# wcq99681-svg/YOLO-AD-Refine

Hardware: AMD Instinct MI355X
Metric: images/sec whole-node (640x640) fwd+bwd, YOLO-AD-Refine-n at 1/2/4/8 GPU (higher is better)
Workload: dtype bf16; 1 GPU; yolo11-701-YOLO-AD-Refine.yaml (n) train step bs=64/GPU 640x640, synthetic COCO-shape labels, TAL+DFL+CIoU/NWD loss, SGD+EMA; global_batch=64, img=640, parallelism=dp1, nms=not in the train step (measured in the inference leg at validator settings)

## Files before the change

### yolo-ad-refine_amd/csrc/adr_mlca.hip

```cpp
#include "adr_common.h"
#include <initializer_list>

namespace adr {

static constexpr int LS = 5;
__device__ __forceinline__ int a_s(int o, int in, int out) { return (int)(((long)o * in) / out); }
__device__ __forceinline__ int a_e(int o, int in, int out) { return (int)(((long)(o + 1) * in + out - 1) / out); }

template <typename T, int VW>
__global__ void __launch_bounds__(256) mlca_pool_kernel(const T* x, int xcs, int H, int W, int C, float* local) {
  __shared__ float red[256 * VW];
  const int p = blockIdx.x, n = blockIdx.y;
  const int i = p / LS, j = p % LS;
  const int hs = a_s(i, H, LS), he = a_e(i, H, LS), ws = a_s(j, W, LS), we = a_e(j, W, LS);
  const int bw = we - ws, cnt = (he - hs) * bw;
  const float inv = 1.f / (float)cnt;
  const int G = C / VW;
  for (int cb = 0; cb < G; cb += 256) {
    const int gn = min(256, G - cb), S = 256 / gn;
    const int cg = cb + threadIdx.x % gn, sp = threadIdx.x / gn, c0 = cg * VW;
    float s[VW];
#pragma unroll
    for (int e = 0; e < VW; ++e) s[e] = 0.f;
    if (sp < S)
// ... 270 lines not shown
    up_att<VW>(att + (long)n * LS * LS * C, C, h, w, H, W, c0, a);
    vload<T, VW>(dout + pix * dcs + c0, g);
#pragma unroll
    for (int e = 0; e < VW; ++e) g[e] *= a[e];
    const float* DL = dlocal + (long)n * LS * LS * C + c0;
    const int bic = h * LS / H, bjc = w * LS / W;
    const int bi0 = H < 2 * LS ? 0 : max(0, bic - 1), bi1 = H < 2 * LS ? LS - 1 : min(LS - 1, bic + 1);
    const int bj0 = W < 2 * LS ? 0 : max(0, bjc - 1), bj1 = W < 2 * LS ? LS - 1 : min(LS - 1, bjc + 1);
    for (int bi = bi0; bi <= bi1; ++bi) {
      const int hs = a_s(bi, H, LS), he = a_e(bi, H, LS);
      if (h < hs || h >= he) continue;
      for (int bj = bj0; bj <= bj1; ++bj) {
        const int ws = a_s(bj, W, LS), we = a_e(bj, W, LS);
        if (w < ws || w >= we) continue;
        const float inv = 1.f / (float)((he - hs) * (we - ws));
        const float* d = DL + (bi * LS + bj) * C;
#pragma unroll
        for (int e = 0; e < VW; ++e) g[e] += d[e] * inv;
      }
    }
    vstore<T, VW>(dy + pix * ocs + c0, g);
  }
}

__global__ void sum_rows_kernel(const float* part, int rows, int cols, float* out0, float* out1) {
  const int c = threadIdx.x;
  if (c >= cols) return;
  const float* p = part + (long)blockIdx.x * cols;
  float s = 0.f;
  for (int r = 0; r < rows; ++r) s += p[(long)r * 2 * cols + c];
  (blockIdx.x ? out1 : out0)[c] = s;
}

}

using namespace adr;

static bool mlca_vec(int dtype, int C, std::initializer_list<long> strides, std::initializer_list<const void*> ptrs) {
  const int vw = dtype == ADR_BF16 ? 8 : 4;
  if (C % vw) return false;
  for (long s : strides)
    if (s % vw) return false;
  for (const void* p : ptrs)
    if ((uintptr_t)p % 16) return false;
  return true;
}
static dim3 mlca_grid(long npix, int dtype, bool v, int C) {
  const int G = C / (v ? (dtype == ADR_BF16 ? 8 : 4) : 1);
  const long rpb = G <= 256 ? 256 / G : 1;
  long b = (npix + rpb - 1) / rpb;
  return dim3((unsigned)(b > 65536 ? 65536 : (b < 1 ? 1 : b)));
}
#define MLCA_DISPATCH(dtype, v, KERN, grid, ...)                                                  \
  do {                                                                                          \
    if ((dtype) == ADR_BF16) {                                                                  \
      using TT = __bf16;                                                                        \
      if (v) hipLaunchKernelGGL((KERN<TT, 8>), grid, dim3(256), 0, st, __VA_ARGS__);            \
      else hipLaunchKernelGGL((KERN<TT, 1>), grid, dim3(256), 0, st, __VA_ARGS__);              \
    } else {                                                                                    \
      using TT = float;                                                                         \
      if (v) hipLaunchKernelGGL((KERN<TT, 4>), grid, dim3(256), 0, st, __VA_ARGS__);            \
      else hipLaunchKernelGGL((KERN<TT, 1>), grid, dim3(256), 0, st, __VA_ARGS__);              \
    }                                                                                           \
  } while (0)

extern "C" int adr_mlca_fwd(int dtype, const void* y, int ycs, const void* res, int rcs, void* out, int ocs, int N,
                            int H, int W, int C, const float* wl, const float* wg, int k, float local_weight,
                            float* local, float* att, float* sig_l, float* sig_g, void* stream) {
  ADR_REQUIRE(k % 2 == 1 && k <= 15, "mlca: k=%d", k);
  ADR_REQUIRE(N >= 1 && H >= 1 && W >= 1 && C >= 1, "mlca_fwd: empty map N=%d H=%d W=%d C=%d", N, H, W, C);
  hipStream_t st = (hipStream_t)stream;
  const bool v = mlca_vec(dtype, C, {ycs, rcs, ocs}, {y, res, out});
  MLCA_DISPATCH(dtype, v, mlca_pool_kernel, dim3(LS * LS, N), (const TT*)y, ycs, H, W, C, local);
  size_t sm = 2 * C * sizeof(float);
  hipLaunchKernelGGL(mlca_att_kernel, dim3(N), dim3(256), sm, st, local, C, wl, wg, k, sig_l, sig_g);
  long natt = (long)N * LS * LS * C;
  hipLaunchKernelGGL(mlca_mix_kernel, dim3(cdiv(natt, 256)), dim3(256), 0, st, sig_l, sig_g, N, C, local_weight, att);
  MLCA_DISPATCH(dtype, v, mlca_apply_kernel, mlca_grid((long)N * H * W, dtype, v, C), (const TT*)y, ycs,
                (const TT*)res, rcs, att, (TT*)out, ocs, N, H, W, C);
  return check_launch("adr_mlca_fwd");
}

extern "C" size_t adr_mlca_bwd_workspace(int N, int C, int k) {
  return ((size_t)N * LS * LS * C * 2 + (size_t)N * k * 2 + (size_t)LS * C) * sizeof(float);
}

extern "C" int adr_mlca_bwd(int dtype, const void* y, int ycs, const void* dout, int dcs, void* dy, int ocs, int N,
                            int H, int W, int C, const float* wl, const float* wg, int k, float local_weight,
                            const float* local, const float* att, const float* sig_l, const float* sig_g, float* dwl,
                            float* dwg, float* ws, size_t ws_bytes, void* stream) {
  ADR_REQUIRE(N >= 1 && H >= 1 && W >= 1 && C >= 1, "mlca_bwd: empty map N=%d H=%d W=%d C=%d", N, H, W, C);
  ADR_REQUIRE(ws_bytes >= adr_mlca_bwd_workspace(N, C, k), "mlca_bwd: workspace too small");
  hipStream_t st = (hipStream_t)stream;
  float* datt = ws;
  float* dlocal = ws + (size_t)N * LS * LS * C;
  float* dwl_part = dlocal + (size_t)N * LS * LS * C;
  float* dwg_part = dwl_part + (size_t)N * k;
  float* S = dwg_part + (size_t)N * k;
  const bool v = mlca_vec(dtype, C, {ycs, dcs, ocs}, {y, dout, dy});
  MLCA_DISPATCH(dtype, v, mlca_bwd_bins_kernel, dim3(LS * LS, N), (const TT*)y, ycs, (const TT*)dout, dcs, H, W, C,
                datt);
  size_t sm = (2 * C + LS * LS * C + 2 * MLCA_NT) * sizeof(float);
  ADR_REQUIRE(sm <= 160 * 1024, "mlca_bwd: C=%d too large for the per-image LDS plan", C);
  hipLaunchKernelGGL(mlca_gsum_kernel, dim3(LS), dim3(256), 0, st, datt, N, C, S);
  hipLaunchKernelGGL(mlca_att_bwd_kernel, dim3(N), dim3(MLCA_NT), sm, st, local, datt, sig_l, sig_g, S, N, C, wl, wg, k,
                     local_weight, dlocal, dwl_part, dwg_part);
  MLCA_DISPATCH(dtype, v, mlca_bwd_y_kernel, mlca_grid((long)N * H * W, dtype, v, C), (const TT*)dout, dcs, att,
                dlocal, (TT*)dy, ocs, N, H, W, C);
  ADR_REQUIRE(k <= 64, "mlca_bwd: kernel size %d", k);
  ADR_REQUIRE((dwl == nullptr) == (dwg == nullptr), "mlca_bwd: dwl and dwg both given or both NULL");
  if (dwl) hipLaunchKernelGGL(sum_rows_kernel, dim3(2), dim3(64), 0, st, dwl_part, N, k, dwl, dwg);
  return check_launch("adr_mlca_bwd");
}
```

### yolo-ad-refine_amd/csrc/adr_conv.hip

```cpp
#include <cstdio>
#include <type_traits>

#include "adr_common.h"

namespace adr {

enum ConvMode { CV_FWD = 0, CV_DGRAD = 1, CV_DGRAD2 = 2 };

struct ConvArgs {
  const __bf16* src;
  const __bf16* wt;
  __bf16* out;
  const float* bias;
  float* stats;
  int n;
  int sh_, sw_, scs, sco, sc;
  int rh, rw, ocs, oco;
  int r, s, str, ph, pw;
  int N;
  int ktot;
  int ntiles;
  int accumulate;
  int src_bytes, wt_bytes;
  const float* escale;
// ... 935 lines not shown
#pragma unroll
      for (int e = 0; e < 8; ++e) nv[e] = (__bf16)((float)nv[e] + (float)ov[e]);
    }
    st16(dst, v);
    if (a.stats) es.add(a, v, yv);
  };
  if constexpr (BST) {
#pragma unroll
    for (int k = 0; k < RPT; ++k) out_row(orow + k * RPP, ypre[k]);
  } else {
    for (int r = orow; r < PIX; r += RPP) out_row(r, ypre[0]);
  }
  if (a.stats) {
    __syncthreads();
#pragma unroll
    for (int e = 0; e < 8; ++e) {
      red[0][orow][oc * 8 + e] = es.s1[e];
      red[1][orow][oc * 8 + e] = es.s2[e];
    }
    __syncthreads();
    if (tid < BN && n0 + tid < a.N) {
      float x1 = 0.f, x2 = 0.f;
      for (int g = 0; g < RPP; ++g) {
        x1 += red[0][g][tid];
        x2 += red[1][g][tid];
      }
      float* s = a.stats + (long)mt * 2 * a.N + n0 + tid;
      s[0] = x1;
      s[a.N] = x2;
    }
  }
}

constexpr int G2_TI = 8, G2_TJ = 8;
template <int TJ>
struct G2Geo {
  static constexpr int NT = 32 * TJ, W = NT / 64;
  static constexpr int HW = TJ + 1, NPIX = (G2_TI + 1) * HW;
  static constexpr int PIX = 4 * G2_TI * TJ;
};
__device__ __forceinline__ void g2_tap(int c, int q, int& t, int& di, int& dj) {
  const int py = c >> 1, px = c & 1;
  const int kh = py ? ((c == 3 ? (q >> 1) : q) ? 2 : 0) : 1;
  const int kw = px ? ((c == 3 ? (q & 1) : q) ? 2 : 0) : 1;
  t = kh * 3 + kw;
  di = py && kh == 0;
  dj = px && kw == 0;
}

template <int TJ, int BN, int XF, bool BST>
__device__ __forceinline__ void dg2_body(const ConvArgs& a) {
  using G = G2Geo<TJ>;
  constexpr int NT = G::NT, W = G::W, HW = G::HW, NPIX = G::NPIX, PIX = G::PIX, DXW = 2 * TJ;
  constexpr int A_TOT = NPIX * (C3_CK / 8), A_CH = (A_TOT + NT - 1) / NT;
  constexpr int B_TOT = 9 * BN * (C3_CK / 8), B_CH = (B_TOT + NT - 1) / NT;
  constexpr int TN = BN / 16, NS = 4;
  constexpr int OPITCH = BN + 8, CPR = BN / 8, RPP = NT / CPR, RPT = PIX / RPP;
  constexpr int SMEM_A = NPIX * C3_LD, SMEM_B = 9 * BN * C3_LD;
  constexpr int SMEM_AB = 2 * (SMEM_A + SMEM_B), SMEM_O = 2 * PIX * OPITCH, SMEM_R = 2 * RPP * BN * 4;
  constexpr int SMEM_BYTES = SMEM_AB > SMEM_O ? (SMEM_AB > SMEM_R ? SMEM_AB : SMEM_R) : (SMEM_O > SMEM_R ? SMEM_O : SMEM_R);
  __shared__ __attribute__((aligned(16))) unsigned char lds_raw[SMEM_BYTES];
  __bf16* As = reinterpret_cast<__bf16*>(lds_raw);
  __bf16* Bs = As + SMEM_A;
  float (*red)[RPP][BN] = reinterpret_cast<float (*)[RPP][BN]>(lds_raw);

  const int tid = threadIdx.x, lane = tid & 63, wave = tid >> 6;
// ... 194 lines not shown
}
template <int BN>
__global__ void __launch_bounds__(256, BN <= 64 ? 4 : 2) conv_bf16_act_kernel(ConvArgs a) { conv_bf16_body<BN, CV_FWD, true>(a); }
template <int TW, bool DG, int BN>
__global__ void __launch_bounds__(256, 3) conv3_kernel(ConvArgs a) { conv3_body<TW, DG, BN, false>(a); }
template <int TW, int BN>
__global__ void __launch_bounds__(256, 3) conv3_act_kernel(ConvArgs a) { conv3_body<TW, false, BN, true>(a); }
template <bool DG, bool EPI>
__global__ void __launch_bounds__(512, 1) conv3w_kernel(ConvArgs a) { conv3_body<16, DG, 128, EPI, XF_NONE, 2>(a); }
template <int BN, int MODE, int XF>
__global__ void __launch_bounds__(256, (XF == XF_BWD && BN == 64) ? 2 : 3) conv_bf16_xf_kernel(ConvArgs a) {
  conv_bf16_body<BN, MODE, false, XF>(a);
}
template <int TW, bool DG, int BN, int XF>
__global__ void __launch_bounds__(256, 2) conv3_xf_kernel(ConvArgs a) { conv3_body<TW, DG, BN, false, XF>(a); }
template <int TJ, int BN, int XF, bool BST>
__global__ void __launch_bounds__(32 * TJ, (XF == XF_BWD && BN == 64) ? 2 : 3) dg2_kernel(ConvArgs a) {
  dg2_body<TJ, BN, XF, BST>(a);
}
template <int BN, int MODE, int XF>
__global__ void __launch_bounds__(256, XF == XF_BWD ? ((BN == 64) ? 2 : 3) : (BN <= 64 ? 4 : 2))
    conv_bf16_bst_kernel(ConvArgs a) {
  conv_bf16_body<BN, MODE, false, XF, true>(a);
}
template <int BN, int KT>
__global__ void __launch_bounds__(256, KT == 256 ? 1 : (KT == 64 && BN <= 64) ? 3 : 2) conv1_bst_kernel(ConvArgs a, int groups) {
  conv1_body<BN, CV_DGRAD, KT, false, XF_NONE, true>(a, groups);
}
template <int TW, int BN, int XF>
__global__ void __launch_bounds__(256, XF == XF_NONE ? 3 : 2) conv3_bst_kernel(ConvArgs a) {
  conv3_body<TW, true, BN, false, XF, 1, true>(a);
}
__global__ void __launch_bounds__(512, 1) conv3w_bst_kernel(ConvArgs a) { conv3_body<16, true, 128, false, XF_NONE, 2, true>(a); }

static int conv3_tw(const adr_conv_desc* d, int red_ch, int out_ch) {
  if (d->r != 3 || d->s != 3 || d->stride_h != 1 || d->pad_h != 1 || red_ch % C3_CK || out_ch % 32) return 0;
  if (d->w % 16 == 0 && d->h >= 8) return 16;
  if (d->w % 8 == 0) return 8;
  return 0;
}
static int conv3_bn(int out_ch) { return out_ch % 64 == 0 ? 64 : 32; }
static int conv3_tiles(const adr_conv_desc* d, int tw, int pix = 128) {
  return d->n * ((d->h + pix / tw - 1) / (pix / tw)) * (d->w / tw);
}
static bool conv3_wide(const adr_conv_desc* d, int tw, int red_ch, int out_ch) {
  return tw == 16 && d->h >= 16 && red_ch >= 128 && out_ch % 128 == 0 &&
         (long)conv3_tiles(d, 16, 256) * (out_ch / 128) >= 512;
}
template <bool DG>
static void launch_conv3(int tw, int bn, const adr_conv_desc* d, ConvArgs& g, hipStream_t st, bool wide = false) {
  if (DG && g.by) {
    if constexpr (!DG) return;
    if (wide) {
      g.ntiles = g.N / 128;
      hipLaunchKernelGGL(conv3w_bst_kernel, dim3(conv3_tiles(d, 16, 256) * g.ntiles), dim3(512), 0, st, g);
      return;
    }
    g.ntiles = g.N / bn;
    dim3 grid(conv3_tiles(d, tw) * g.ntiles);
#define ADR_C3B(TW_, BN_)                                                                                   \
  do {                                                                                                      \
    if (g.xs) hipLaunchKernelGGL((conv3_bst_kernel<TW_, BN_, XF_BWD>), grid, dim3(256), 0, st, g);          \
    else hipLaunchKernelGGL((conv3_bst_kernel<TW_, BN_, XF_NONE>), grid, dim3(256), 0, st, g);              \
  } while (0)
    if (bn == 64) {
      if (tw == 16) ADR_C3B(16, 64);
      else ADR_C3B(8, 64);
    } else {
      if (tw == 16) ADR_C3B(16, 32);
      else ADR_C3B(8, 32);
    }
#undef ADR_C3B
    return;
  }
  if (wide) {
    g.ntiles = g.N / 128;
    dim3 grid(conv3_tiles(d, 16, 256) * g.ntiles);
    if (!DG && g.escale) hipLaunchKernelGGL((conv3w_kernel<false, true>), grid, dim3(512), 0, st, g);
    else hipLaunchKernelGGL((conv3w_kernel<DG, false>), grid, dim3(512), 0, st, g);
    return;
  }
// ... 136 lines not shown
      case 16: ADR_C1(16, 256); break;
      case 32: ADR_C1(32, 256); break;
      default: ADR_C1(64, 256); break;
    }
  }
#undef ADR_C1
}

static int conv_pick_bn(int n) { return n <= 16 ? 16 : n <= 32 ? 32 : n <= 64 ? 64 : 128; }

static int conv_check(const adr_conv_desc* d) {
  ADR_REQUIRE(d && d->n > 0 && d->h > 0 && d->w > 0 && d->c > 0 && d->k > 0 && d->r > 0 && d->s > 0,
              "conv: bad geometry");
  ADR_REQUIRE(d->dtype == ADR_BF16, "conv (bf16 engine): dtype %d", d->dtype);
  ADR_REQUIRE(d->c % 8 == 0 && d->k % 8 == 0, "conv: C (%d) and K (%d) must be multiples of 8", d->c, d->k);
  ADR_REQUIRE(d->x_cstride % 8 == 0 && d->x_coff % 8 == 0 && d->y_cstride % 8 == 0 && d->y_coff % 8 == 0,
              "conv: channel views must be 16-byte aligned");
  ADR_REQUIRE(d->x_cstride >= d->x_coff + d->c && d->y_cstride >= d->y_coff + d->k, "conv: view exceeds stride");
  ADR_REQUIRE(d->stride_h == d->stride_w, "conv: anisotropic stride");
  const int ho = (d->h + 2 * d->pad_h - d->r) / d->stride_h + 1, wo = (d->w + 2 * d->pad_w - d->s) / d->stride_w + 1;
  ADR_REQUIRE(ho == d->ho && wo == d->wo, "conv: output size mismatch (%dx%d vs %dx%d)", d->ho, d->wo, ho, wo);
  ADR_REQUIRE((long)d->n * d->h * d->w * d->x_cstride < (1l << 30) && (long)d->n * d->ho * d->wo * d->y_cstride < (1l << 30)
              && (long)d->k * d->c * d->r * d->s < (1l << 30), "conv: tensor exceeds 2^30 elements (32-bit buffer offsets)");
  return ADR_OK;
}

struct ConvPlan {
  int tw;
  int wide;
  int bn;
  int mode;
  int kt;
  int dg2;
};
static int dg2_mode() {
  const char* e = getenv("ADR_DG2H");
  return e ? atoi(e) : 1;
}
static ConvPlan conv_plan(const adr_conv_desc* d, bool dgrad, bool xf = false) {
  ConvPlan p{0, 0, 0, dgrad ? (d->stride_h == 2 ? CV_DGRAD2 : CV_DGRAD) : CV_FWD};
  const int red = dgrad ? d->k : d->c, out = dgrad ? d->c : d->k;
  const long g2_area = (long)((d->ho + G2_TI - 1) / G2_TI * G2_TI) * ((d->wo + G2_TJ - 1) / G2_TJ * G2_TJ);
  if (p.mode == CV_DGRAD2 && d->r == 3 && d->s == 3 && d->pad_h == 1 && d->pad_w == 1 && red % C3_CK == 0 &&
      out % 16 == 0 && (out <= 64 || out % 64 == 0) && dg2_mode() &&
      (dg2_mode() == 2 || g2_area * 100 <= 115l * d->ho * d->wo)) {
    p.dg2 = G2_TJ;
    p.bn = out % 64 == 0 ? 64 : out % 32 == 0 ? 32 : 16;
    p.kt = 0;
    return p;
  }
  if (p.mode != CV_DGRAD2) p.tw = conv3_tw(d, red, out);
  p.wide = p.tw && !xf && conv3_wide(d, p.tw, red, out);
  p.bn = p.tw ? conv3_bn(out) : ((d->r * d->s == 1 || xf) && out > 64) ? 64 : conv_pick_bn(out);
  {
    const long rows = dgrad ? (long)d->n * d->h * d->w : (long)d->n * d->ho * d->wo;
    const long grid128 = (rows + CBM - 1) / CBM * ((out + 127) / 128);
    if (!p.tw && p.bn == 128 && grid128 < 1024) p.bn = 64;
  }
  p.kt = 0;
  const bool c1 = !p.tw && p.mode != CV_DGRAD2 && d->r == 1 && d->s == 1 && d->stride_h == 1 && d->pad_h == 0 &&
                  d->pad_w == 0;
  if (c1 && (!xf || !dgrad) && red <= (dgrad && p.bn <= 64 ? 256 : 128))
    p.kt = red <= 64 ? 64 : red <= 128 ? 128 : 256;
  return p;
}

static int xf_args(const adr_bnact_xf* xf, bool bwd, int red, int n, int sh, int sw, ConvArgs& g) {
  ADR_REQUIRE(xf && xf->scale && xf->shift && xf->out && (xf->act == ACT_NONE || xf->act == ACT_SILU),
              "conv bnact: scale / shift / side output / act (none or silu)");
  ADR_REQUIRE(red <= XMAXC, "conv bnact: %d reduction channels (table holds %d)", red, XMAXC);
  ADR_REQUIRE(xf->out_cstride >= red && xf->out_cstride % 8 == 0 && ((uintptr_t)xf->out & 15) == 0,
              "conv bnact: side output view");
  g.xs = xf->scale; g.xt = xf->shift; g.xact = xf->act;
  g.xo = (__bf16*)xf->out; g.xocs = xf->out_cstride;
  if (bwd) {
    ADR_REQUIRE(xf->y && xf->A && xf->B && xf->Cc && xf->y_cstride >= red && xf->y_cstride % 8 == 0 &&
                    ((uintptr_t)xf->y & 15) == 0,
                "conv bnact (dgrad): y view and A / B / Cc coefficients");
    ADR_REQUIRE((long)n * sh * sw * xf->y_cstride < (1l << 30), "conv bnact: y exceeds 2^30 elements");
    g.xy = (const __bf16*)xf->y; g.xycs = xf->y_cstride; g.xy_bytes = (int)(2l * n * sh * sw * xf->y_cstride);
    g.xA = xf->A; g.xB = xf->B; g.xC = xf->Cc;
  }
  return ADR_OK;
}

}

using namespace adr;

static int conv_fwd_impl(const adr_conv_desc* d, const void* x, const void* w, const float* bias, void* y,
                         float* stats, int accumulate, const float* escale, const float* eshift, int eact,
                         void* stream, const adr_bnact_xf* xf = nullptr) {
  int rc = conv_check(d);
  if (rc) return rc;
  ConvArgs g{};
  if (xf) {
    ADR_REQUIRE(!escale, "conv fwd bnact: no eval epilogue");
    rc = xf_args(xf, false, d->c, d->n, d->h, d->w, g);
    if (rc) return rc;
  }
  g.src = (const __bf16*)x; g.wt = (const __bf16*)w; g.out = (__bf16*)y; g.bias = bias; g.stats = stats;
  g.escale = escale; g.eshift = eshift; g.eact = escale ? eact : 0;
  g.n = d->n; g.sh_ = d->h; g.sw_ = d->w; g.scs = d->x_cstride; g.sco = d->x_coff; g.sc = d->c;
  g.rh = d->ho; g.rw = d->wo; g.ocs = d->y_cstride; g.oco = d->y_coff;
  g.r = d->r; g.s = d->s; g.str = d->stride_h; g.ph = d->pad_h; g.pw = d->pad_w;
  g.N = d->k; g.ktot = d->r * d->s * d->c; g.accumulate = accumulate;
  g.src_bytes = (int)(2l * d->n * d->h * d->w * d->x_cstride);
  g.wt_bytes = (int)(2l * g.N * g.ktot);
  const ConvPlan pl = conv_plan(d, false, xf != nullptr);
  if (pl.tw) {
    launch_conv3<false>(pl.tw, pl.bn, d, g, (hipStream_t)stream, pl.wide);
    return check_launch("adr_conv2d_fwd_bf16");
  }
  const int bn = pl.bn;
  g.ntiles = cdiv(g.N, bn);
  if (pl.kt) {
    launch_conv1<CV_FWD>(bn, pl.kt, (long)d->n * d->ho * d->wo, g, (hipStream_t)stream);
    return check_launch("adr_conv2d_fwd_bf16");
  }
  dim3 grid(cdiv((long)d->n * d->ho * d->wo, CBM) * g.ntiles);
  launch_conv<CV_FWD>(bn, grid, g, (hipStream_t)stream);
  return check_launch("adr_conv2d_fwd_bf16");
}

extern "C" int adr_conv2d_fwd_bf16(const adr_conv_desc* d, const void* x, const void* w, const float* bias, void* y,
                                   float* stats, int accumulate, void* stream) {
  return conv_fwd_impl(d, x, w, bias, y, stats, accumulate, nullptr, nullptr, 0, stream);
}

extern "C" int adr_conv2d_fwd_bf16_act(const adr_conv_desc* d, const void* x, const void* w, const float* scale,
                                       const float* shift, int act, void* y, void* stream) {
  ADR_REQUIRE(scale && shift && act >= ACT_NONE && act <= ACT_HSWISH, "conv fwd act: scale/shift/act");
  return conv_fwd_impl(d, x, w, nullptr, y, nullptr, 0, scale, shift, act, stream);
}

static int conv_dgrad_impl(const adr_conv_desc* d, const void* dy, const void* w_crsk, const float* bias, void* dx,
                           int accumulate, const void* addend, int adcs, void* stream,
                           const adr_bnact_xf* xf = nullptr, const adr_bn_bstat* bst = nullptr,
                           float* stats = nullptr) {
  int rc = conv_check(d);
  if (rc) return rc;
  ConvArgs g{};
  if (xf) {
    rc = xf_args(xf, true, d->k, d->n, d->ho, d->wo, g);
    if (rc) return rc;
  }
  if (bst) {
    ADR_REQUIRE(stats && bst->y && bst->scale && bst->shift && (bst->act == ACT_NONE || bst->act == ACT_SILU),
                "conv dgrad bstat: stats / y / scale / shift / act (none or silu)");
    ADR_REQUIRE(bst->y_cstride >= d->c && bst->y_cstride % 8 == 0 && ((uintptr_t)bst->y & 15) == 0 &&
                    ((uintptr_t)bst->scale & 15) == 0 && ((uintptr_t)bst->shift & 15) == 0,
                "conv dgrad bstat: 16-byte aligned y view / coefficients");
    ADR_REQUIRE((long)d->n * d->h * d->w * bst->y_cstride < (1l << 30), "conv dgrad bstat: y exceeds 2^30 elements");
    g.by = (const __bf16*)bst->y; g.bycs = bst->y_cstride; g.bact = bst->act; g.bs = bst->scale; g.bt = bst->shift;
  }
  g.src = (const __bf16*)dy; g.wt = (const __bf16*)w_crsk; g.out = (__bf16*)dx; g.bias = bias;
  g.stats = bst ? stats : nullptr;
  g.addend = (const __bf16*)addend; g.adcs = adcs;
  g.n = d->n; g.sh_ = d->ho; g.sw_ = d->wo; g.scs = d->y_cstride; g.sco = d->y_coff; g.sc = d->k;
  g.rh = d->h; g.rw = d->w; g.ocs = d->x_cstride; g.oco = d->x_coff;
  g.r = d->r; g.s = d->s; g.str = d->stride_h; g.ph = d->pad_h; g.pw = d->pad_w;
  g.N = d->c; g.ktot = d->r * d->s * d->k; g.accumulate = accumulate;
  g.src_bytes = (int)(2l * d->n * d->ho * d->wo * d->y_cstride);
  g.wt_bytes = (int)(2l * g.N * g.ktot);
  ADR_REQUIRE(d->stride_h == 1 || d->stride_h == 2, "conv dgrad (bf16 engine): stride %d", d->stride_h);
  const ConvPlan pl = conv_plan(d, true, xf != nullptr);
  const int bn = pl.bn;
  g.ntiles = cdiv(g.N, bn);
  hipStream_t st = (hipStream_t)stream;
  if (pl.dg2) {
    launch_dg2(bn, d, g, st);
  } else if (pl.mode == CV_DGRAD2) {
    dim3 grid(cdiv((long)d->n * ((d->h + 1) / 2) * ((d->w + 1) / 2), CBM) * g.ntiles, 1, 4);
    launch_conv<CV_DGRAD2>(bn, grid, g, st);
  } else if (pl.tw) {
    launch_conv3<true>(pl.tw, pl.bn, d, g, st, pl.wide);
  } else if (pl.kt) {
    launch_conv1<CV_DGRAD>(bn, pl.kt, (long)d->n * d->h * d->w, g, st);
  } else {
    dim3 grid(cdiv((long)d->n * d->h * d->w, CBM) * g.ntiles);
    launch_conv<CV_DGRAD>(bn, grid, g, st);
  }
  return check_launch("adr_conv2d_dgrad_bf16");
}

extern "C" int adr_conv2d_dgrad_bf16(const adr_conv_desc* d, const void* dy, const void* w_crsk, const float* bias,
                                     void* dx, int accumulate, void* stream) {
  return conv_dgrad_impl(d, dy, w_crsk, bias, dx, accumulate, nullptr, 0, stream);
}

extern "C" int adr_conv2d_dgrad_bf16_add(const adr_conv_desc* d, const void* dy, const void* w_crsk, void* dx,
                                         int accumulate, const void* addend, int addend_cstride, void* stream) {
  ADR_REQUIRE(addend && addend_cstride >= d->c && addend_cstride % 8 == 0 && ((uintptr_t)addend & 15) == 0,
              "conv dgrad add: addend must be a 16-byte aligned NHWC view with channel stride >= C");
  return conv_dgrad_impl(d, dy, w_crsk, nullptr, dx, accumulate, addend, addend_cstride, stream);
}

extern "C" int adr_conv2d_dgrad_bf16_bnact(const adr_conv_desc* d, const void* dz, const void* w_crsk, void* dx,
                                           int accumulate, const void* addend, int addend_cstride,
                                           const adr_bnact_xf* xf, void* stream) {
  ADR_REQUIRE(xf, "conv dgrad bnact: xf");
  if (addend)
    ADR_REQUIRE(addend_cstride >= d->c && addend_cstride % 8 == 0 && ((uintptr_t)addend & 15) == 0,
                "conv dgrad bnact: addend view");
// ... 8 lines not shown
  if (addend)
    ADR_REQUIRE(addend_cstride >= d->c && addend_cstride % 8 == 0 && ((uintptr_t)addend & 15) == 0,
                "conv dgrad bstat: addend view");
  return conv_dgrad_impl(d, dy, w_crsk, nullptr, dx, accumulate, addend, addend_cstride, stream, xf, bs, stats);
}

extern "C" int adr_conv2d_fwd_bf16_bnact(const adr_conv_desc* d, const void* y, const void* w, void* out,
                                         float* stats, const adr_bnact_xf* xf, void* stream) {
  ADR_REQUIRE(xf, "conv fwd bnact: xf");
  return conv_fwd_impl(d, y, w, nullptr, out, stats, 0, nullptr, nullptr, 0, stream, xf);
}

extern "C" int adr_conv2d_bf16_xf_reuse(const adr_conv_desc* d, int dgrad) {
  const ConvPlan pl = conv_plan(d, dgrad != 0, true);
  if (dgrad) {
    const char* es = getenv("ADR_XF_STREAM");
    const char* eg = getenv("ADR_XF_DG2");
    const char* e3 = getenv("ADR_XF_CONV3");
    if (!(es && atoi(es)) && conv_plan(d, true, false).kt > 0 && pl.kt == 0) return 1 << 20;
    if (!(eg && atoi(eg)) && pl.dg2) return 1 << 20;
    if (!(e3 && atoi(e3)) && pl.tw) return 1 << 20;
  }
  const int out = dgrad ? d->c : d->k;
  const int nt = pl.tw ? out / pl.bn : cdiv(out, pl.bn);
  if (pl.dg2) return nt * 100 * (G2_TI + 1) * (pl.dg2 + 1) / (G2_TI * pl.dg2);
  if (pl.tw) return nt * 100 * (128 / pl.tw + 2) * (pl.tw + 2) / 128;
  const int taps = d->r * d->s;
  if (!dgrad) return nt * 100 * taps / (d->stride_h * d->stride_w);
  return nt * 100 * taps;
}

static int fwd_stat_tiles(const adr_conv_desc* d, bool xf) {
  const ConvPlan pl = conv_plan(d, false, xf);
  if (pl.tw) return pl.wide ? conv3_tiles(d, 16, 256) : conv3_tiles(d, pl.tw);
  if (pl.kt) return conv1_groups((long)d->n * d->ho * d->wo, cdiv(d->k, pl.bn), pl.kt, pl.bn);
  return cdiv((long)d->n * d->ho * d->wo, CBM);
}

extern "C" int adr_conv2d_fwd_bf16_stat_tiles(const adr_conv_desc* d) { return fwd_stat_tiles(d, false); }

extern "C" int adr_conv2d_dgrad_bf16_stat_tiles(const adr_conv_desc* d, int xf) {
  const ConvPlan pl = conv_plan(d, true, xf != 0);
  if (pl.dg2) return dg2_tiles(d);
  if (pl.mode == CV_DGRAD2) return 4 * cdiv((long)d->n * ((d->h + 1) / 2) * ((d->w + 1) / 2), CBM);
  if (pl.tw) return pl.wide ? conv3_tiles(d, 16, 256) : conv3_tiles(d, pl.tw);
  if (pl.kt) return conv1_groups((long)d->n * d->h * d->w, cdiv(d->c, pl.bn), pl.kt, pl.bn);
  return cdiv((long)d->n * d->h * d->w, CBM);
}

extern "C" int adr_conv2d_fwd_bf16_bnact_stat_tiles(const adr_conv_desc* d) { return fwd_stat_tiles(d, true); }

extern "C" int adr_conv2d_bf16_kernel_symbol(const adr_conv_desc* d, int dgrad, char* buf, int len) {
  ADR_REQUIRE(d && buf && len >= 64, "conv kernel symbol: bad arguments");
  const bool dg = (dgrad & 1) != 0, xf = (dgrad & 2) != 0;
  const bool bst = dg && (dgrad & 4) != 0;
  const ConvPlan pl = conv_plan(d, dg, xf);
  if (pl.dg2) {
    snprintf(buf, len, "_ZN3adr10dg2_kernelILi%dELi%dELi%dELb%dEEEvNS_8ConvArgsE", pl.dg2, pl.bn, xf ? XF_BWD : XF_NONE,
             bst ? 1 : 0);
    return ADR_OK;
  }
  if (bst) {
    if (pl.tw && pl.wide && !xf)
      snprintf(buf, len, "_ZN3adr17conv3w_bst_kernelENS_8ConvArgsE");
    else if (pl.tw)
      snprintf(buf, len, "_ZN3adr16conv3_bst_kernelILi%dELi%dELi%dEEEvNS_8ConvArgsE", pl.tw, pl.bn, xf ? XF_BWD : XF_NONE);
    else if (pl.kt && !xf)
      snprintf(buf, len, "_ZN3adr16conv1_bst_kernelILi%dELi%dEEEvNS_8ConvArgsEi", pl.bn, pl.kt);
    else
      snprintf(buf, len, "_ZN3adr20conv_bf16_bst_kernelILi%dELi%dELi%dEEEvNS_8ConvArgsE", pl.bn, pl.mode,
               xf ? XF_BWD : XF_NONE);
    return ADR_OK;
  }
  if (xf && pl.tw)
    snprintf(buf, len, "_ZN3adr15conv3_xf_kernelILi%dELb%dELi%dELi%dEEEvNS_8ConvArgsE", pl.tw, dg ? 1 : 0, pl.bn,
             dg ? XF_BWD : XF_FWD);
  else if (xf)
    snprintf(buf, len, "_ZN3adr19conv_bf16_xf_kernelILi%dELi%dELi%dEEEvNS_8ConvArgsE", pl.bn, pl.mode,
             dg ? XF_BWD : XF_FWD);
  else if (pl.tw && pl.wide)
    snprintf(buf, len, "_ZN3adr13conv3w_kernelILb%dELb0EEEvNS_8ConvArgsE", dg ? 1 : 0);
  else if (pl.tw)
    snprintf(buf, len, "_ZN3adr12conv3_kernelILi%dELb%dELi%dEEEvNS_8ConvArgsE", pl.tw, dg ? 1 : 0, pl.bn);
  else if (pl.kt && xf)
    snprintf(buf, len, "_ZN3adr15conv1_xf_kernelILi%dELi%dEEEvNS_8ConvArgsEi", pl.bn, pl.kt);
  else if (pl.kt)
    snprintf(buf, len, "_ZN3adr12conv1_kernelILi%dELi%dELi%dEEEvNS_8ConvArgsEi", pl.bn, pl.mode, pl.kt);
  else
    snprintf(buf, len, "_ZN3adr16conv_bf16_kernelILi%dELi%dEEEvNS_8ConvArgsE", pl.bn, pl.mode);
  return ADR_OK;
}
// ... 1 lines not shown
```

Before: 3313 images/s.

## Add per-image tiled MLCA backward kernels with LDS-cached attention and bin tables

Adds two alternative MLCA backward kernels, enabled by default via ADR_MLCA_FUSED when C<=320 and H,W<=256. The bins kernel precomputes adaptive-pool bin boundaries and reciprocals into shared tables. The dy kernel splits each image into blocks of pixels, stages only the needed rows of att and dlocal into LDS, and reads them from there instead of global memory. The aim is to cut repeated index division and global reads of attention in the upsample/backward; it adds larger blocks (512 threads), extra LDS use, and env-var/getenv overhead per call.

```diff
diff --git a/yolo-ad-refine_amd/csrc/adr_mlca.hip b/yolo-ad-refine_amd/csrc/adr_mlca.hip
--- a/yolo-ad-refine_amd/csrc/adr_mlca.hip
+++ b/yolo-ad-refine_amd/csrc/adr_mlca.hip
@@ -326,6 +326,136 @@
   (blockIdx.x ? out1 : out0)[c] = s;
 }
 
+static constexpr int MLCA_MAXHW = 256;
+static constexpr int MLCA_MAXC = 320;
+static constexpr int MLCA_NTF = 512;
+
+struct MlcaTabs {
+  unsigned char is[MLCA_MAXHW], ie[MLCA_MAXHW], js[MLCA_MAXHW], je[MLCA_MAXHW];
+  float inv[LS * LS + 1];
+  float pinv[LS * LS];
+};
+__device__ __forceinline__ void mlca_fill_tabs(MlcaTabs& tb, int H, int W) {
+  const int t0 = threadIdx.x;
+  for (int t = t0; t < H; t += blockDim.x) {
+    tb.is[t] = (unsigned char)a_s(t, LS, H);
+    tb.ie[t] = (unsigned char)a_e(t, LS, H);
+  }
+  for (int t = t0; t < W; t += blockDim.x) {
+    tb.js[t] = (unsigned char)a_s(t, LS, W);
+    tb.je[t] = (unsigned char)a_e(t, LS, W);
+  }
+  if (t0 >= 1 && t0 <= LS * LS) tb.inv[t0] = 1.f / (float)t0;
+  if (t0 < LS * LS) {
+    const int i = t0 / LS, j = t0 % LS;
+    tb.pinv[t0] = 1.f / (float)((a_e(i, H, LS) - a_s(i, H, LS)) * (a_e(j, W, LS) - a_s(j, W, LS)));
+  }
+}
+
+template <int VW>
+__device__ __forceinline__ void up_att_tab(const float* A, int C, const MlcaTabs& tb, int h, int w, int c0,
+                                           float* out) {
+  const int is = tb.is[h], ie = tb.ie[h], js = tb.js[w], je = tb.je[w];
+#pragma unroll
+  for (int e = 0; e < VW; ++e) out[e] = 0.f;
+  for (int i = is; i < ie; ++i)
+    for (int j = js; j < je; ++j) {
+      const float* a = A + (i * LS + j) * C + c0;
+#pragma unroll
+      for (int e = 0; e < VW; ++e) out[e] += a[e];
+    }
+  const float inv = tb.inv[(ie - is) * (je - js)];
+#pragma unroll
+  for (int e = 0; e < VW; ++e) out[e] *= inv;
+}
+
+template <typename T, int VW>
+__global__ void __launch_bounds__(256) mlca_bwd_bins_win_kernel(const T* y, int ycs, const T* dout, int dcs, int H,
+                                                                int W, int C, float* datt) {
+  __shared__ float red[256 * VW];
+  __shared__ MlcaTabs tb;
+  const int p = blockIdx.x, n = blockIdx.y;
+  const int bi = p / LS, bj = p % LS;
+  const int hs = a_s(bi, H, LS), he = a_e(bi, H, LS), ws = a_s(bj, W, LS), we = a_e(bj, W, LS);
+  const int h0 = max(0, hs - 1), w0 = max(0, ws - 1), w1 = min(W, we + 1);
+  const int rw = w1 - w0, bw = we - ws;
+  mlca_fill_tabs(tb, H, W);
+  __syncthreads();
+  const int G = C / VW;
+  const int S = 256 / G;
+  const int cg = threadIdx.x % G, sp = threadIdx.x / G, c0 = cg * VW;
+  float s[VW];
+#pragma unroll
+  for (int e = 0; e < VW; ++e) s[e] = 0.f;
+  if (sp < S)
+    for (int h = hs; h < he; ++h) {
+      const int base = (h - h0) * rw + (ws - w0);
+      const int nh = tb.ie[h] - tb.is[h];
+      int d = (sp - base) % S;
+      if (d < 0) d += S;
+      for (; d < bw; d += S) {
+        const int w = ws + d;
+        const float inv = tb.inv[nh * (tb.je[w] - tb.js[w])];
+        const long pix = ((long)n * H + h) * W + w;
+        float dv[VW], v[VW];
+        vload<T, VW>(dout + pix * dcs + c0, dv);
+        vload<T, VW>(y + pix * ycs + c0, v);
+#pragma unroll
+        for (int e = 0; e < VW; ++e) s[e] += dv[e] * v[e] * inv;
+      }
+    }
+#pragma unroll
+  for (int e = 0; e < VW; ++e) red[threadIdx.x * VW + e] = s[e];
+  __syncthreads();
+  for (int c = threadIdx.x; c < C; c += 256) {
+    float t = 0.f;
+    for (int r = 0; r < S; ++r) t += red[r * C + c];
+    datt[((long)n * LS * LS + p) * C + c] = t;
+  }
+}
+
+template <typename T, int VW>
+__global__ void __launch_bounds__(MLCA_NTF) mlca_bwd_y_img_kernel(const T* dout, int dcs, const float* att,
+                                                                  const float* dlocal, T* dy, int ocs, int N, int H,
+                                                                  int W, int C) {
+  extern __shared__ __align__(16) float A[];
+  __shared__ MlcaTabs tb;
+  float* DL = A + LS * LS * C;
+  const int n = blockIdx.y, b = blockIdx.x, nb = gridDim.x, tid = threadIdx.x;
+  const int HW = H * W;
+  const int p0 = (int)((long)b * HW / nb), p1 = (int)((long)(b + 1) * HW / nb);
+  mlca_fill_tabs(tb, H, W);
+  __syncthreads();
+  const int lo = tb.is[p0 / W] * LS * C, hi = tb.ie[(p1 - 1) / W] * LS * C;
+  const long abase = (long)n * LS * LS * C;
+  for (int it = lo + 4 * tid; it < hi; it += 4 * MLCA_NTF) {
+    *reinterpret_cast<float4*>(A + it) = *reinterpret_cast<const float4*>(att + abase + it);
+    *reinterpret_cast<float4*>(DL + it) = *reinterpret_cast<const float4*>(dlocal + abase + it);
+  }
+  __syncthreads();
+  const int G = C / VW, rpb = MLCA_NTF / G;
+  const int cg = tid % G, r0 = tid / G, c0 = cg * VW;
+  if (r0 >= rpb) return;
+  for (int q = p0 + r0; q < p1; q += rpb) {
+    const int h = q / W, w = q - h * W;
+    const long pix = (long)n * HW + q;
+    float a[VW], g[VW];
+    up_att_tab<VW>(A, C, tb, h, w, c0, a);
+    vload<T, VW>(dout + pix * dcs + c0, g);
+#pragma unroll
+    for (int e = 0; e < VW; ++e) g[e] *= a[e];
+    const int is = tb.is[h], ie = tb.ie[h], js = tb.js[w], je = tb.je[w];
+    for (int bi = is; bi < ie; ++bi)
+      for (int bj = js; bj < je; ++bj) {
+        const float inv = tb.pinv[bi * LS + bj];
+        const float* d = DL + (bi * LS + bj) * C + c0;
+#pragma unroll
+        for (int e = 0; e < VW; ++e) g[e] += d[e] * inv;
+      }
+    vstore<T, VW>(dy + pix * ocs + c0, g);
+  }
+}
+
 }
 
 using namespace adr;
@@ -357,6 +487,31 @@
       else hipLaunchKernelGGL((KERN<TT, 1>), grid, dim3(256), 0, st, __VA_ARGS__);              \
     }                                                                                           \
   } while (0)
+#define MLCA_DISPATCH_IMG(dtype, KERN, grid, block, smem, ...)                                   \
+  do {                                                                                          \
+    if ((dtype) == ADR_BF16) {                                                                  \
+      using TT = __bf16;                                                                        \
+      hipLaunchKernelGGL((KERN<TT, 8>), grid, dim3(block), smem, st, __VA_ARGS__);              \
+    } else {                                                                                    \
+      using TT = float;                                                                         \
+      hipLaunchKernelGGL((KERN<TT, 4>), grid, dim3(block), smem, st, __VA_ARGS__);              \
+    }                                                                                           \
+  } while (0)
+
+static bool mlca_fused(bool v, int H, int W, int C) {
+  const char* e = getenv("ADR_MLCA_FUSED");
+  return (e ? atoi(e) != 0 : true) && v && C <= MLCA_MAXC && H <= MLCA_MAXHW && W <= MLCA_MAXHW;
+}
+#ifndef MLCA_IPT
+#define MLCA_IPT 4
+#endif
+static int mlca_bpi(int H, int W, int C, int dtype) {
+  const int ipt = MLCA_IPT;
+  const long items = (long)H * W * (C / (dtype == ADR_BF16 ? 8 : 4));
+  long b = (items + (long)MLCA_NTF * ipt - 1) / ((long)MLCA_NTF * ipt);
+  if (b > (long)H * W) b = (long)H * W;
+  return (int)(b < 1 ? 1 : (b > 4096 ? 4096 : b));
+}
 
 extern "C" int adr_mlca_fwd(int dtype, const void* y, int ycs, const void* res, int rcs, void* out, int ocs, int N,
                             int H, int W, int C, const float* wl, const float* wg, int k, float local_weight,
@@ -392,15 +547,25 @@
   float* dwg_part = dwl_part + (size_t)N * k;
   float* S = dwg_part + (size_t)N * k;
   const bool v = mlca_vec(dtype, C, {ycs, dcs, ocs}, {y, dout, dy});
-  MLCA_DISPATCH(dtype, v, mlca_bwd_bins_kernel, dim3(LS * LS, N), (const TT*)y, ycs, (const TT*)dout, dcs, H, W, C,
-                datt);
+  const bool fz = mlca_fused(v, H, W, C);
+  if (fz)
+    MLCA_DISPATCH_IMG(dtype, mlca_bwd_bins_win_kernel, dim3(LS * LS, N), 256, 0, (const TT*)y, ycs, (const TT*)dout,
+                      dcs, H, W, C, datt);
+  else
+    MLCA_DISPATCH(dtype, v, mlca_bwd_bins_kernel, dim3(LS * LS, N), (const TT*)y, ycs, (const TT*)dout, dcs, H, W, C,
+                  datt);
   size_t sm = (2 * C + LS * LS * C + 2 * MLCA_NT) * sizeof(float);
   ADR_REQUIRE(sm <= 160 * 1024, "mlca_bwd: C=%d too large for the per-image LDS plan", C);
   hipLaunchKernelGGL(mlca_gsum_kernel, dim3(LS), dim3(256), 0, st, datt, N, C, S);
   hipLaunchKernelGGL(mlca_att_bwd_kernel, dim3(N), dim3(MLCA_NT), sm, st, local, datt, sig_l, sig_g, S, N, C, wl, wg, k,
                      local_weight, dlocal, dwl_part, dwg_part);
-  MLCA_DISPATCH(dtype, v, mlca_bwd_y_kernel, mlca_grid((long)N * H * W, dtype, v, C), (const TT*)dout, dcs, att,
-                dlocal, (TT*)dy, ocs, N, H, W, C);
+  if (fz)
+    MLCA_DISPATCH_IMG(dtype, mlca_bwd_y_img_kernel, dim3(mlca_bpi(H, W, C, dtype), N), MLCA_NTF,
+                      (size_t)2 * LS * LS * C * sizeof(float), (const TT*)dout, dcs, att, dlocal, (TT*)dy, ocs, N, H, W,
+                      C);
+  else
+    MLCA_DISPATCH(dtype, v, mlca_bwd_y_kernel, mlca_grid((long)N * H * W, dtype, v, C), (const TT*)dout, dcs, att,
+                  dlocal, (TT*)dy, ocs, N, H, W, C);
   ADR_REQUIRE(k <= 64, "mlca_bwd: kernel size %d", k);
   ADR_REQUIRE((dwl == nullptr) == (dwg == nullptr), "mlca_bwd: dwl and dwg both given or both NULL");
   if (dwl) hipLaunchKernelGGL(sum_rows_kernel, dim3(2), dim3(64), 0, st, dwl_part, N, k, dwl, dwg);
```

After: 3323 images/s, median of 6. Within noise of the previous version (+0.3%).

## Add narrow-channel 3x3 conv kernel that holds full reduction in LDS

Applied to the files above, without the earlier changes.

Adds a dedicated 3x3 stride-1 conv kernel for layers with at most 32 input and output channels, used for both forward and data-gradient passes. It loads the whole halo tile and the full 9*C weight matrix into LDS once, then runs a single MFMA loop over the packed tap-channel reduction. This removes the multi-stage K loop and the channel-padding overhead that the generic conv3 or implicit-GEMM paths pay on thin layers. It applies only when there are enough tiles, and the old path can be restored with an environment variable. In exchange it adds a new code path with its own epilogue and stats handling, dynamic LDS sizing, and the risk of lower occupancy.

```diff
diff --git a/yolo-ad-refine_amd/csrc/adr_conv.hip b/yolo-ad-refine_amd/csrc/adr_conv.hip
--- a/yolo-ad-refine_amd/csrc/adr_conv.hip
+++ b/yolo-ad-refine_amd/csrc/adr_conv.hip
@@ -991,6 +991,187 @@
   }
 }
 
+__host__ __device__ constexpr int n3_pitch(int sc) { return ((sc >> 3) | 1) << 3; }
+__host__ __device__ constexpr int n3_kp(int sc) { return (9 * sc + 31) & ~31; }
+constexpr int N3_NPIX = 180;
+static int n3_lds_bytes(int sc, int bn, bool stats) {
+  const int ab = 2 * (N3_NPIX * n3_pitch(sc) + bn * (n3_kp(sc) + 8));
+  const int img = 2 * 128 * (bn + 8), red = stats ? 2 * (256 / (bn / 8)) * bn * 4 : 0;
+  return ab > img ? (ab > red ? ab : red) : (img > red ? img : red);
+}
+
+template <int TW, bool DG, int BN, bool BST>
+__device__ __forceinline__ void conv3n_body(const ConvArgs& a) {
+  static_assert(!BST || DG, "BSTAT: data gradients only");
+  constexpr int PIX = 128, TH = PIX / TW, HWW = TW + 2, NPIX = (TH + 2) * HWW;
+  static_assert(NPIX == N3_NPIX, "thin conv3: halo size");
+  constexpr int A_CH = (NPIX * 4 + 255) / 256;
+  constexpr int B_CH = (BN * (n3_kp(32) / 8) + 255) / 256;
+  constexpr int TM = 2, TN = BN / 16;
+  constexpr int OPITCH = BN + 8, CPR = BN / 8, RPP = 256 / CPR, RPT = PIX / RPP;
+  extern __shared__ __attribute__((aligned(16))) unsigned char n3_lds[];
+  const int sc = a.sc, cq = sc >> 3, AP = n3_pitch(sc), KP = n3_kp(sc), BP = KP + 8, kpc = KP >> 3;
+  __bf16* As = reinterpret_cast<__bf16*>(n3_lds);
+  __bf16* Bs = As + NPIX * AP;
+  float (*red)[RPP][BN] = reinterpret_cast<float (*)[RPP][BN]>(n3_lds);
+
+  const int tid = threadIdx.x, lane = tid & 63, wave = tid >> 6;
+  const int H = a.rh, W = a.rw;
+  const int tx = W / TW, ty = (H + TH - 1) / TH;
+  const int mt = xcd_block(blockIdx.x, gridDim.x);
+  const int img = mt / (tx * ty), trem = mt - img * (tx * ty);
+  const int y0 = (trem / tx) * TH, x0 = (trem - (trem / tx) * tx) * TW;
+
+  constexpr unsigned OOR = 0x7FFFFFF0u;
+  const __amdgpu_buffer_rsrc_t src_rs = __builtin_amdgcn_make_buffer_rsrc((void*)a.src, (short)0, a.src_bytes, 0x00020000);
+  const __amdgpu_buffer_rsrc_t wt_rs = __builtin_amdgcn_make_buffer_rsrc((void*)a.wt, (short)0, a.wt_bytes, 0x00020000);
+  u32x4 ra[A_CH], rb[B_CH];
+#pragma unroll
+  for (int i = 0; i < A_CH; ++i) {
+    const int e = tid + 256 * i, q = e / cq, c = e - q * cq, hy = q / HWW, hx = q - hy * HWW;
+    const int gy = y0 - 1 + hy, gx = x0 - 1 + hx;
+    const bool ok = e < NPIX * cq && gy >= 0 && gy < a.sh_ && gx >= 0 && gx < a.sw_;
+    ra[i] = __builtin_amdgcn_raw_buffer_load_b128(
+        src_rs, ok ? (unsigned)(((img * a.sh_ + gy) * a.sw_ + gx) * a.scs + a.sco + c * 8) * 2u : OOR, 0, 0);
+  }
+#pragma unroll
+  for (int i = 0; i < B_CH; ++i) {
+    const int e = tid + 256 * i, row = e / kpc, j = e - row * kpc;
+    const bool ok = row < BN && row < a.N && j * 8 < a.ktot;
+    rb[i] = __builtin_amdgcn_raw_buffer_load_b128(wt_rs, ok ? (unsigned)(row * a.ktot + j * 8) * 2u : OOR, 0, 0);
+  }
+#pragma unroll
+  for (int i = 0; i < A_CH; ++i) {
+    const int e = tid + 256 * i, q = e / cq, c = e - q * cq;
+    if (e < NPIX * cq) st16(&As[q * AP + c * 8], ra[i]);
+  }
+#pragma unroll
+  for (int i = 0; i < B_CH; ++i) {
+    const int e = tid + 256 * i, row = e / kpc, j = e - row * kpc;
+    if (row < BN) st16(&Bs[row * BP + j * 8], rb[i]);
+  }
+  __syncthreads();
+
+  const int l15 = lane & 15, kq = lane >> 4;
+  int fq[TM];
+#pragma unroll
+  for (int i = 0; i < TM; ++i) {
+    const int p = wave * 32 + i * 16 + l15;
+    fq[i] = (p / TW) * HWW + (p % TW);
+  }
+  f32x4 acc[TM][TN];
+#pragma unroll
+  for (int i = 0; i < TM; ++i)
+#pragma unroll
+    for (int j = 0; j < TN; ++j) acc[i][j] = (f32x4){0.f, 0.f, 0.f, 0.f};
+  int tap = 0, c0 = kq * 8;
+  while (c0 >= sc) {
+    c0 -= sc;
+    ++tap;
+  }
+  const u32x4 zero = {0u, 0u, 0u, 0u};
+  for (int kk = 0; kk < KP; kk += 32) {
+    const bool tok = tap < 9;
+    const int kh = (tap * 11) >> 5, kw = tap - 3 * kh;
+    const int dq = !tok ? 0 : DG ? (2 - kh) * HWW + (2 - kw) : kh * HWW + kw;
+    u32x4 fa[TM], fb[TN];
+#pragma unroll
+    for (int i = 0; i < TM; ++i) {
+      fa[i] = *reinterpret_cast<const u32x4*>(&As[(fq[i] + dq) * AP + c0]);
+      if (!tok) fa[i] = zero;
+    }
+#pragma unroll
+    for (int j = 0; j < TN; ++j) fb[j] = *reinterpret_cast<const u32x4*>(&Bs[(j * 16 + l15) * BP + kk + kq * 8]);
+#pragma unroll
+    for (int i = 0; i < TM; ++i)
+#pragma unroll
+      for (int j = 0; j < TN; ++j)
+        acc[i][j] = __builtin_amdgcn_mfma_f32_16x16x32_bf16(*reinterpret_cast<const bf16x8*>(&fa[i]),
+                                                            *reinterpret_cast<const bf16x8*>(&fb[j]), acc[i][j], 0, 0, 0);
+    c0 += 32;
+    while (c0 >= sc) {
+      c0 -= sc;
+      ++tap;
+    }
+  }
+  __syncthreads();
+
+  __bf16* Os = reinterpret_cast<__bf16*>(n3_lds);
+  const bool epi = a.escale != nullptr;
+#pragma unroll
+  for (int j = 0; j < TN; ++j) {
+    const int col = j * 16 + l15;
+    const bool cok = col < a.N;
+    const float b = (a.bias && cok) ? a.bias[col] : 0.f;
+    const float es = epi && cok ? a.escale[col] : 1.f;
+    const float eb = epi && cok ? a.eshift[col] + b : b;
+#pragma unroll
+    for (int i = 0; i < TM; ++i)
+#pragma unroll
+      for (int e = 0; e < 4; ++e)
+        Os[(wave * 32 + i * 16 + 4 * kq + e) * OPITCH + col] =
+            (__bf16)(epi ? epi_act(a.eact, fmaf(acc[i][j][e], es, eb)) : acc[i][j][e] + b);
+  }
+  const int oc = tid % CPR, orow = tid / CPR;
+  const bool col_ok = oc * 8 < a.N;
+  u32x4 ypre[BST ? RPT : 1];
+  if constexpr (BST) {
+#pragma unroll
+    for (int k = 0; k < RPT; ++k) {
+      const int r = orow + k * RPP, y = y0 + r / TW;
+      ypre[k] = (y < H && col_ok) ? ld16(a.by + ((long)(img * H + y) * W + x0 + r % TW) * a.bycs + oc * 8)
+                                  : u32x4{0u, 0u, 0u, 0u};
+    }
+  }
+  __syncthreads();
+  EpiStats<BST> es;
+  es.init(a, col_ok, oc * 8);
+  auto out_row = [&](int r, const u32x4& yv) {
+    const int y = y0 + r / TW;
+    if (y >= H || !col_ok) return;
+    u32x4 v = *reinterpret_cast<const u32x4*>(&Os[r * OPITCH + oc * 8]);
+    const long pix = (long)(img * H + y) * W + x0 + r % TW;
+    __bf16* dst = a.out + pix * a.ocs + a.oco + oc * 8;
+    if (DG && a.addend) {
+      const u32x4 q = ld16(a.addend + pix * a.adcs + oc * 8);
+      const u32x4 o = a.accumulate ? ld16(dst) : u32x4{0u, 0u, 0u, 0u};
+      const __bf16 *qv = reinterpret_cast<const __bf16*>(&q), *ov = reinterpret_cast<const __bf16*>(&o);
+      __bf16* nv = reinterpret_cast<__bf16*>(&v);
+#pragma unroll
+      for (int e = 0; e < 8; ++e) nv[e] = (__bf16)((float)nv[e] + (float)ov[e] + (float)qv[e]);
+    } else if (a.accumulate) {
+      const u32x4 o = ld16(dst);
+      const __bf16* ov = reinterpret_cast<const __bf16*>(&o);
+      __bf16* nv = reinterpret_cast<__bf16*>(&v);
+#pragma unroll
+      for (int e = 0; e < 8; ++e) nv[e] = (__bf16)((float)nv[e] + (float)ov[e]);
+    }
+    st16(dst, v);
+    if (a.stats) es.add(a, v, yv);
+  };
+#pragma unroll
+  for (int k = 0; k < RPT; ++k) out_row(orow + k * RPP, ypre[BST ? k : 0]);
+  if (a.stats) {
+    __syncthreads();
+#pragma unroll
+    for (int e = 0; e < 8; ++e) {
+      red[0][orow][oc * 8 + e] = es.s1[e];
+      red[1][orow][oc * 8 + e] = es.s2[e];
+    }
+    __syncthreads();
+    if (tid < BN && tid < a.N) {
+      float x1 = 0.f, x2 = 0.f;
+      for (int g = 0; g < RPP; ++g) {
+        x1 += red[0][g][tid];
+        x2 += red[1][g][tid];
+      }
+      float* s = a.stats + (long)mt * 2 * a.N + tid;
+      s[0] = x1;
+      s[a.N] = x2;
+    }
+  }
+}
+
 constexpr int G2_TI = 8, G2_TJ = 8;
 template <int TJ>
 struct G2Geo {
@@ -1251,6 +1432,8 @@
   conv3_body<TW, true, BN, false, XF, 1, true>(a);
 }
 __global__ void __launch_bounds__(512, 1) conv3w_bst_kernel(ConvArgs a) { conv3_body<16, true, 128, false, XF_NONE, 2, true>(a); }
+template <int TW, bool DG, int BN, bool BST>
+__global__ void __launch_bounds__(256, 4) conv3_narrow(ConvArgs a) { conv3n_body<TW, DG, BN, BST>(a); }
 
 static int conv3_tw(const adr_conv_desc* d, int red_ch, int out_ch) {
   if (d->r != 3 || d->s != 3 || d->stride_h != 1 || d->pad_h != 1 || red_ch % C3_CK || out_ch % 32) return 0;
@@ -1266,6 +1449,40 @@
   return tw == 16 && d->h >= 16 && red_ch >= 128 && out_ch % 128 == 0 &&
          (long)conv3_tiles(d, 16, 256) * (out_ch / 128) >= 512;
 }
+static int thin3_mode() {
+  const char* e = getenv("ADR_THIN3");
+  return e ? atoi(e) : 1;
+}
+constexpr int N3_MIN_TILES = 256;
+static int thin3_tw(const adr_conv_desc* d, int red_ch, int out_ch) {
+  if (d->r != 3 || d->s != 3 || d->stride_h != 1 || d->pad_h != 1 || d->pad_w != 1 || d->w % 8) return 0;
+  if (red_ch > 32 || out_ch > 32 || conv3_tw(d, red_ch, out_ch)) return 0;
+  const int mode = thin3_mode();
+  if (!mode) return 0;
+  const int tw = (d->w % 16 == 0 && d->h >= 8) ? 16 : 8;
+  if (mode != 2 && conv3_tiles(d, tw) < N3_MIN_TILES) return 0;
+  return tw;
+}
+template <bool DG>
+static void launch_conv3n(int tw, int bn, const adr_conv_desc* d, ConvArgs& g, hipStream_t st) {
+  g.ntiles = 1;
+  const dim3 grid(conv3_tiles(d, tw));
+  const int lds = n3_lds_bytes(g.sc, bn, g.stats != nullptr);
+#define ADR_N3(TW_, BN_)                                                                                        \
+  do {                                                                                                          \
+    if (DG && g.by) hipLaunchKernelGGL((conv3_narrow<TW_, true, BN_, true>), grid, dim3(256), lds, st, g);      \
+    else hipLaunchKernelGGL((conv3_narrow<TW_, DG, BN_, false>), grid, dim3(256), lds, st, g);                  \
+  } while (0)
+  if (bn == 32) {
+    if (tw == 16) ADR_N3(16, 32);
+    else ADR_N3(8, 32);
+  } else {
+    if (tw == 16) ADR_N3(16, 16);
+    else ADR_N3(8, 16);
+  }
+#undef ADR_N3
+}
+
 template <bool DG>
 static void launch_conv3(int tw, int bn, const adr_conv_desc* d, ConvArgs& g, hipStream_t st, bool wide = false) {
   if (DG && g.by) {
@@ -1468,6 +1685,7 @@
   int mode;
   int kt;
   int dg2;
+  int thin;
 };
 static int dg2_mode() {
   const char* e = getenv("ADR_DG2H");
@@ -1486,6 +1704,10 @@
     return p;
   }
   if (p.mode != CV_DGRAD2) p.tw = conv3_tw(d, red, out);
+  if (p.mode != CV_DGRAD2 && !xf && (p.thin = thin3_tw(d, red, out))) {
+    p.bn = out <= 16 ? 16 : 32;
+    return p;
+  }
   p.wide = p.tw && !xf && conv3_wide(d, p.tw, red, out);
   p.bn = p.tw ? conv3_bn(out) : ((d->r * d->s == 1 || xf) && out > 64) ? 64 : conv_pick_bn(out);
   {
@@ -1544,6 +1766,10 @@
   g.src_bytes = (int)(2l * d->n * d->h * d->w * d->x_cstride);
   g.wt_bytes = (int)(2l * g.N * g.ktot);
   const ConvPlan pl = conv_plan(d, false, xf != nullptr);
+  if (pl.thin) {
+    launch_conv3n<false>(pl.thin, pl.bn, d, g, (hipStream_t)stream);
+    return check_launch("adr_conv2d_fwd_bf16");
+  }
   if (pl.tw) {
     launch_conv3<false>(pl.tw, pl.bn, d, g, (hipStream_t)stream, pl.wide);
     return check_launch("adr_conv2d_fwd_bf16");
@@ -1606,6 +1832,8 @@
   hipStream_t st = (hipStream_t)stream;
   if (pl.dg2) {
     launch_dg2(bn, d, g, st);
+  } else if (pl.thin) {
+    launch_conv3n<true>(pl.thin, bn, d, g, st);
   } else if (pl.mode == CV_DGRAD2) {
     dim3 grid(cdiv((long)d->n * ((d->h + 1) / 2) * ((d->w + 1) / 2), CBM) * g.ntiles, 1, 4);
     launch_conv<CV_DGRAD2>(bn, grid, g, st);
@@ -1680,6 +1908,7 @@
 
 static int fwd_stat_tiles(const adr_conv_desc* d, bool xf) {
   const ConvPlan pl = conv_plan(d, false, xf);
+  if (pl.thin) return conv3_tiles(d, pl.thin);
   if (pl.tw) return pl.wide ? conv3_tiles(d, 16, 256) : conv3_tiles(d, pl.tw);
   if (pl.kt) return conv1_groups((long)d->n * d->ho * d->wo, cdiv(d->k, pl.bn), pl.kt, pl.bn);
   return cdiv((long)d->n * d->ho * d->wo, CBM);
@@ -1690,6 +1919,7 @@
 extern "C" int adr_conv2d_dgrad_bf16_stat_tiles(const adr_conv_desc* d, int xf) {
   const ConvPlan pl = conv_plan(d, true, xf != 0);
   if (pl.dg2) return dg2_tiles(d);
+  if (pl.thin) return conv3_tiles(d, pl.thin);
   if (pl.mode == CV_DGRAD2) return 4 * cdiv((long)d->n * ((d->h + 1) / 2) * ((d->w + 1) / 2), CBM);
   if (pl.tw) return pl.wide ? conv3_tiles(d, 16, 256) : conv3_tiles(d, pl.tw);
   if (pl.kt) return conv1_groups((long)d->n * d->h * d->w, cdiv(d->c, pl.bn), pl.kt, pl.bn);
@@ -1705,6 +1935,11 @@
   const ConvPlan pl = conv_plan(d, dg, xf);
   if (pl.dg2) {
     snprintf(buf, len, "_ZN3adr10dg2_kernelILi%dELi%dELi%dELb%dEEEvNS_8ConvArgsE", pl.dg2, pl.bn, xf ? XF_BWD : XF_NONE,
+             bst ? 1 : 0);
+    return ADR_OK;
+  }
+  if (pl.thin) {
+    snprintf(buf, len, "_ZN3adr12conv3_narrowILi%dELb%dELi%dELb%dEEEvNS_8ConvArgsE", pl.thin, dg ? 1 : 0, pl.bn,
              bst ? 1 : 0);
     return ADR_OK;
   }
```

Result: no change. 3320 images/s before, 3346 images/s after (median of 6 runs) (+0.8%).
